# Alandroid/img-compression-mps

Measured on AMD Instinct MI355X. Metric: Mvoxels/s compress+reconstruct, 256^3 fp32, bond chi=64; SSIM vs ref, higher is better.
Workload: dtype f32

## Files before the change

img-compression-mps_amd/_lib.py:

```python
import ctypes as C
import os

_HERE = os.path.dirname(os.path.abspath(__file__))
LIB_PATH = os.path.join(_HERE, "libndmps_hip.so")

OK, EINVAL, EHIP, ENOCONV, EWORKSPACE, ETEAM = 0, -1, -2, -3, -4, -5

i64 = C.c_int64
p_i64 = C.POINTER(C.c_int64)
p_f64 = C.POINTER(C.c_double)
p_f32 = C.POINTER(C.c_float)
p_int = C.POINTER(C.c_int)
vp = C.c_void_p

SIGNATURES = {
    "ndmps_version": (C.c_int, []),
    "ndmps_last_error": (C.c_char_p, []),
    "ndmps_device_count": (C.c_int, []),
    "ndmps_streams_create": (C.c_int, [C.c_int, C.POINTER(vp), C.POINTER(C.c_int)]),
    "ndmps_streams_destroy": (C.c_int, [C.c_int, C.POINTER(vp)]),
    "ndmps_profile_enable": (C.c_int, [C.c_int]),
    "ndmps_profile_collect": (C.c_int, [C.c_int, p_f64, p_i64, p_i64]),
    "ndmps_plan_create": (C.c_int, [C.POINTER(vp), C.c_int, p_i64, C.c_int, p_i64]),
    "ndmps_plan_create_reversed": (C.c_int, [C.POINTER(vp), C.c_int, p_i64, C.c_int, p_i64]),
# ... 92 lines not shown
    "ndmps_potrf_scratch_elems": (i64, [i64]),
    "ndmps_potrf_lower_f64": (C.c_int, [vp, i64, vp, C.POINTER(C.c_int), vp]),
    "ndmps_syevd_topk_workspace_bytes": (i64, [i64, C.c_int, i64]),
    "ndmps_syevd_topk_stamps_offset": (i64, [i64, C.c_int, i64]),
    "ndmps_syevd_topk_values_f64": (C.c_int, [C.c_int, vp, i64, p_i64, vp, i64, vp, i64, i64, vp, i64, vp]),
    "ndmps_syevd_topk_vectors_f64": (C.c_int, [C.c_int, p_i64, p_i64, i64, vp, i64, p_int, vp]),
    "ndmps_syevd_topk_vectors_auto_f64": (C.c_int, [C.c_int, p_i64, i64, C.c_double, vp, vp, i64, vp, vp, i64, vp]),
    "ndmps_syevd_topk_recover_f64": (C.c_int, [C.c_int, p_i64, i64, vp, i64, p_int, vp]),
    "ndmps_syevd_topk_set_team": (C.c_int, [C.c_int]),
    "ndmps_syevd_topk_set_streamed": (C.c_int, [C.c_int]),
    "ndmps_syevd_topk_team_fallbacks": (i64, []),
    "ndmps_syevd_topk_team_slots": (C.c_int, [i64]),
    "ndmps_syevd_topk_note_team_fallback": (C.c_int, []),
    "ndmps_debug_inject_team_abort": (C.c_int, [C.c_int]),
    "ndmps_debug_lane_sums_f64": (C.c_int, [vp, vp, vp]),
    "ndmps_tt_sweep_pads_cores": (C.c_int, [C.c_int, p_i64, i64]),
    "ndmps_tt_sweep_async_ints": (i64, [C.c_int, C.c_int]),
    "ndmps_tt_sweep_async_doubles": (i64, [C.c_int, C.c_int, p_i64, i64]),
    "ndmps_tt_sweep_batched_fused_begin_f32": (C.c_int, [C.c_int, C.POINTER(vp), C.c_int, p_i64, C.c_double, i64,
                                                         C.POINTER(vp), p_i64, p_i64, vp, vp, vp, vp, vp, i64,
                                                         vp, i64, vp, vp, vp]),
    "ndmps_tt_sweep_finish": (C.c_int, [C.c_int, C.c_int, p_i64, i64, vp, vp, p_i64, p_f64, p_i64]),
    "ndmps_tt_sweep_batched_workspace_bytes": (i64, [C.c_int, C.c_int, p_i64, i64]),
    "ndmps_tt_sweep_batched_f32": (C.c_int, [C.c_int, C.POINTER(vp), C.c_int, p_i64, C.c_double, i64,
                                             C.POINTER(vp), p_i64, p_i64, p_f64, p_i64, vp, i64, vp]),
    "ndmps_tt_layout": (C.c_int, [C.c_int, p_i64, i64, p_i64, p_i64, p_i64, p_i64]),
    "ndmps_tt_sweep_f32": (C.c_int, [vp, C.c_int, p_i64, C.c_double, i64, vp, p_i64, p_i64, p_f64,
                                     p_i64, vp, i64, vp]),
    "ndmps_compress_bond_workspace_bytes": (i64, [i64, i64, i64, i64, i64]),
    "ndmps_compress_bond_f32": (C.c_int, [vp, vp, i64, i64, i64, i64, i64, C.c_double, i64, vp, vp,
# ... 102 lines not shown
```

img-compression-mps_amd/csrc/gemm.hip:

```cpp
#include <stdlib.h>

#include <algorithm>

#include <mutex>
#include <type_traits>

#include "common.h"

namespace {

typedef float f32x16 __attribute__((ext_vector_type(16)));
typedef double f64x4 __attribute__((ext_vector_type(4)));

template <typename T>
struct Mfma;

template <>
struct Mfma<float> {
  static constexpr int MT = 32;
  static constexpr int KS = 2;
  static constexpr int NACC = 16;
  typedef f32x16 acc_t;
  static __device__ __forceinline__ acc_t mma(float a, float b, acc_t c) {
    return __builtin_amdgcn_mfma_f32_32x32x2f32(a, b, c, 0, 0, 0);
// ... 829 lines not shown
    Gb[pr * n + pc] = s;
    Gb[pc * n + pr] = s;
  }
}

constexpr int G128_LD = 128 + 16;
constexpr int G128_PANEL = GW_KB * G128_LD;
constexpr size_t kGram128Lds = (size_t)4 * G128_PANEL * sizeof(float);
constexpr int kGram128MaxBatch = 48;

struct Gram128Geom {
  int tiles_1d, n_off, n_diag;
  int slabs_off, slabs_diag;
  int64_t rows_off, rows_diag;
  int slots;
  int xcd, members, groups_per_matrix, groups_total;
};
struct Gram128Ptrs {
  const void* a[kGram128MaxBatch];
};

template <int ROLE>
__device__ __forceinline__ void gram128_load(const float* pa, const float* pb, int s, double (&av)[4], double (&bv)[4]) {
  const int off = 4 * s * G128_LD;
  if (ROLE == 1) {
#pragma unroll
    for (int a = 0; a < 4; ++a) av[a] = bv[a] = (double)pa[off + 16 * a];
  } else {
#pragma unroll
    for (int a = 0; a < (ROLE == 2 ? 2 : 4); ++a) av[a] = (double)pa[off + 16 * a];
#pragma unroll
    for (int b = 0; b < 4; ++b) bv[b] = (double)pb[off + 16 * b];
  }
}
template <int ROLE>
// ... 3 lines not shown
#pragma unroll
    for (int b = 0; b < 4; ++b)
      if (ROLE != 1 || a <= b) acc[4 * a + b] = __builtin_amdgcn_mfma_f64_16x16x4f64(av[a], bv[b], acc[4 * a + b], 0, 0, 0);
}
template <int ROLE>
__device__ __forceinline__ void gram128_chunk(const float* pa, const float* pb, f64x4 (&acc)[16]) {
  double av[2][4], bv[2][4];
  gram128_load<ROLE>(pa, pb, 0, av[0], bv[0]);
#pragma unroll
  for (int s = 0; s < GW_KB / 4; ++s) {
    if (s + 1 < GW_KB / 4) gram128_load<ROLE>(pa, pb, s + 1, av[(s + 1) & 1], bv[(s + 1) & 1]);
    gram128_mfma<ROLE>(av[s & 1], bv[s & 1], acc);
  }
}

template <typename TIN, int MODE>
__global__ void __launch_bounds__(256, 2)
gram128_kernel(Gram128Ptrs ptrs, int64_t m, int64_t n, int64_t lda, double* __restrict__ partial, Gram128Geom g,
               int vec_ok, const int64_t* __restrict__ row_off, const int64_t* __restrict__ col_off) {
  extern __shared__ __attribute__((aligned(16))) float g128_lds[];
  int id = blockIdx.x, vol = blockIdx.y;
  if (g.xcd) {
    const int x = blockIdx.x & 7, q = blockIdx.x >> 3;
    const int group = (q / g.members) * 8 + x, mem = q % g.members;
    if (group >= g.groups_total) return;
    vol = group / g.groups_per_matrix;
    const int sp = group % g.groups_per_matrix;
    if (g.xcd == 2) {
      id = mem < g.n_off ? mem * g.slabs_off + sp : g.n_off * g.slabs_off + (mem - g.n_off) * g.slabs_diag + sp;
    } else if (mem < 2 * g.n_off) {
      const int sl = 2 * sp + mem / g.n_off;
      if (sl >= g.slabs_off) return;
      id = (mem % g.n_off) * g.slabs_off + sl;
    } else {
      id = g.n_off * g.slabs_off + (mem - 2 * g.n_off) * g.slabs_diag + sp;
    }
  }
  const TIN* __restrict__ A = static_cast<const TIN*>(ptrs.a[vol]);
  int ti, tj, slab;
  int64_t rows;
  if (id < g.n_off * g.slabs_off) {
    int t = id / g.slabs_off;
    slab = id % g.slabs_off;
    rows = g.rows_off;
    ti = 0;
    while (t >= g.tiles_1d - 1 - ti) {
      t -= g.tiles_1d - 1 - ti;
      ++ti;
    }
    tj = ti + 1 + t;
  } else {
    const int t = (id - g.n_off * g.slabs_off) / g.slabs_diag;
    slab = (id - g.n_off * g.slabs_off) % g.slabs_diag;
    rows = g.rows_diag;
    ti = tj = t;
  }
  const bool diag = ti == tj;
  const int64_t i0 = (int64_t)ti * 128, j0 = (int64_t)tj * 128;
  const int64_t r_begin = (int64_t)slab * rows;
  const int64_t r_end = min(m, r_begin + rows);

  const int tid = threadIdx.x, lane = tid & 63, wave = tid >> 6;
  const int lr = lane >> 4, lc = lane & 15;

  float4 pi[4], pj[4];
  int64_t coli = 0, colj = 0, ro[4] = {0, 0, 0, 0};
  auto row_offsets = [&](int64_t r0) {
    if (MODE == 2 || (MODE == 0 && row_off)) {
#pragma unroll
      for (int v = 0; v < 4; ++v) {
        const int64_t row = r0 + (tid + 256 * v) / 32;
        ro[v] = row < r_end ? row_off[row] : 0;
      }
    }
  };
  if (MODE == 2 || (MODE == 0 && row_off)) {
    const int c4 = (tid % 32) * 4;
    if (i0 + c4 + 3 < n) coli = col_off[i0 + c4];
    if (j0 + c4 + 3 < n) colj = col_off[j0 + c4];
  }
  auto fetch = [&](int64_t r0) {
    if constexpr (MODE != 0) {
      const int c4 = (tid % 32) * 4;
#pragma unroll
      for (int v = 0; v < 4; ++v) {
        const TIN* src = MODE == 2 ? A + ro[v] + coli : A + (r0 + (tid + 256 * v) / 32) * lda + i0 + c4;
        pi[v] = load4_as_f32(src);
      }
      if (!diag) {
#pragma unroll
        for (int v = 0; v < 4; ++v) {
          const TIN* src = MODE == 2 ? A + ro[v] + colj : A + (r0 + (tid + 256 * v) / 32) * lda + j0 + c4;
          pj[v] = load4_as_f32(src);
        }
      }
      return;
    }
#pragma unroll
    for (int v = 0; v < 4; ++v) {
      const int e = tid + 256 * v;
      const int rr = e / 32, c4 = (e % 32) * 4;
      const int64_t row = r0 + rr;
      float4 x = make_float4(0.f, 0.f, 0.f, 0.f), y = x;
      if (row < r_end && row_off) {
        const TIN* base = A + ro[v];
        if (i0 + c4 + 3 < n) x = load4_as_f32(base + coli);
        if (!diag && j0 + c4 + 3 < n) y = load4_as_f32(base + colj);
      } else if (row < r_end) {
        const TIN* base = A + row * lda;
        if (vec_ok && i0 + c4 + 3 < n) x = load4_as_f32(base + i0 + c4);
        else {
          if (i0 + c4 + 0 < n) x.x = (float)base[i0 + c4 + 0];
// ... 102 lines not shown
    base = g.n_off * g.slabs_off + (t - g.n_off) * g.slabs_diag;
    count = g.slabs_diag;
  }
  const int64_t r = (int64_t)ti * 128 + e / 128, c = (int64_t)tj * 128 + e % 128;
  if (r >= n || c >= n || (ti == tj && c < r)) return;
  const double* src = partial + ((int64_t)blockIdx.z * g.slots + base) * (128 * 128) + e;
  double s = 0.0;
  int sl = 0;
  for (; sl + 4 <= count; sl += 4) {
    const double v0 = src[(int64_t)(sl + 0) * 16384], v1 = src[(int64_t)(sl + 1) * 16384];
    const double v2 = src[(int64_t)(sl + 2) * 16384], v3 = src[(int64_t)(sl + 3) * 16384];
    s = (((s + v0) + v1) + v2) + v3;
  }
  for (; sl < count; ++sl) s += src[(int64_t)sl * 16384];
  double* Gb = G + (int64_t)blockIdx.z * stride_G;
  const int64_t pr = perm ? perm[r] : r, pc = perm ? perm[c] : c;
  Gb[pr * n + pc] = s;
  Gb[pc * n + pr] = s;
}

template <typename TIN>
__global__ void __launch_bounds__(256)
gram_small_kernel(const TIN* __restrict__ A, int64_t m, int n, int64_t lda, double* __restrict__ partial,
                  int vec_ok) {
  __shared__ double red[4][36];
  double acc[36];
#pragma unroll
  for (int i = 0; i < 36; ++i) acc[i] = 0.0;
  const int64_t stride = (int64_t)gridDim.x * 256;
  for (int64_t r = (int64_t)blockIdx.x * 256 + threadIdx.x; r < m; r += stride) {
// ... 338 lines not shown
inline bool gram_use_128(int64_t m, int64_t n) { return n >= 128 && m >= 256; }

Gram128Geom gram128_geometry(int64_t m, int64_t n, int batch) {
  Gram128Geom g;
  g.tiles_1d = (int)ndmps::ceil_div(n, 128);
  g.n_off = g.tiles_1d * (g.tiles_1d - 1) / 2;
  g.n_diag = g.tiles_1d;
  const double weight = g.n_off + 0.625 * g.n_diag;
  const double want = 2.0 * ndmps::kNumCU * (batch > 1 ? 12.0 : 1.0) / std::max(batch, 1) / weight;
  const int64_t floor_rows = batch > 1 ? 512 : 128;
  int64_t s_off = std::max<int64_t>(1, std::min<int64_t>((int64_t)(want + 0.5), std::max<int64_t>(m / floor_rows, 1)));
  g.rows_off = ndmps::round_up(ndmps::ceil_div(m, s_off), GW_KB);
  g.rows_diag = ndmps::round_up((g.rows_off * 8 + 4) / 5, GW_KB);
  g.slabs_off = (int)ndmps::ceil_div(m, g.rows_off);
  g.slabs_diag = (int)ndmps::ceil_div(m, g.rows_diag);
  g.xcd = 0;
  g.members = g.groups_per_matrix = g.groups_total = 0;
  const char* xe = getenv("NDMPS_GRAM_XCD");
  const int xmode = xe ? atoi(xe) : 0;
  if (batch > 1 && g.tiles_1d >= 2 && g.slabs_off >= 4 && xmode == 1) {
    g.rows_diag = 2 * g.rows_off;
    g.slabs_diag = (int)ndmps::ceil_div(m, g.rows_diag);
    g.xcd = 1;
    g.members = 2 * g.n_off + g.n_diag;
    g.groups_per_matrix = g.slabs_diag;
    g.groups_total = batch * g.groups_per_matrix;
  } else if (batch > 1 && g.tiles_1d >= 2 && g.slabs_off >= 4 && xmode == 2) {
    const int64_t s2 = std::max<int64_t>(1, (int64_t)(g.slabs_off * weight / (g.n_off + g.n_diag) + 0.5));
    g.rows_off = g.rows_diag = ndmps::round_up(ndmps::ceil_div(m, s2), GW_KB);
    g.slabs_off = g.slabs_diag = (int)ndmps::ceil_div(m, g.rows_off);
    g.xcd = 2;
    g.members = g.n_off + g.n_diag;
    g.groups_per_matrix = g.slabs_off;
    g.groups_total = batch * g.groups_per_matrix;
  }
  g.slots = g.n_off * g.slabs_off + g.n_diag * g.slabs_diag;
  return g;
}

inline int64_t gram128_workspace(int64_t m, int64_t n, int batch) {
  return (int64_t)batch * gram128_geometry(m, n, batch).slots * 128 * 128 * (int64_t)sizeof(double) + 256;
}

int gram128_opt_in() {
  static std::mutex mu;
  static bool done[64] = {};
  int dev = 0;
  NDMPS_CHECK_HIP(hipGetDevice(&dev));
  std::lock_guard<std::mutex> lock(mu);
  if (dev < 0 || dev >= 64 || done[dev]) return NDMPS_OK;
#define NDMPS_GRAM128_OPT_IN(T, MODE)                                                                          \
  NDMPS_CHECK_HIP(hipFuncSetAttribute(reinterpret_cast<const void*>(&gram128_kernel<T, MODE>),                 \
                                      hipFuncAttributeMaxDynamicSharedMemorySize, (int)kGram128Lds))
  NDMPS_GRAM128_OPT_IN(float, 0);
  NDMPS_GRAM128_OPT_IN(float, 1);
  NDMPS_GRAM128_OPT_IN(float, 2);
  NDMPS_GRAM128_OPT_IN(__bf16, 0);
  NDMPS_GRAM128_OPT_IN(__bf16, 1);
  NDMPS_GRAM128_OPT_IN(__bf16, 2);
#undef NDMPS_GRAM128_OPT_IN
  done[dev] = true;
  return NDMPS_OK;
}

template <typename TIN>
int gram128_batched(int batch, const TIN* const* h_A, int64_t m, int64_t n, int64_t lda, double* d_G, int64_t stride_G,
                    void* d_ws, int64_t ws_bytes, hipStream_t s, const int64_t* d_row_off, const int64_t* d_col_off,
                    const int32_t* d_perm = nullptr) {
  NDMPS_REQUIRE(batch >= 1 && h_A && d_G && gram_use_128(m, n) && lda >= n && stride_G >= n * n,
                "bad batched Gram argument (batch=%d m=%lld n=%lld)", batch, (long long)m, (long long)n);
  const int64_t need = gram128_workspace(m, n, batch);
  if (!d_ws || ws_bytes < need) {
    ndmps::set_error("Gram workspace too small: %lld < %lld", (long long)ws_bytes, (long long)need);
    return NDMPS_EWORKSPACE;
  }
  NDMPS_TRY(gram128_opt_in());
  const Gram128Geom g = gram128_geometry(m, n, batch);
  int vec_ok = (lda % 4 == 0 && n % 4 == 0) ? 1 : 0;
  for (int b = 0; b < batch; ++b) {
    NDMPS_REQUIRE(h_A[b], "NULL Gram operand %d", b);
    if ((uintptr_t)h_A[b] % (4 * sizeof(TIN)) != 0) vec_ok = 0;
  }
  if (d_row_off)
    NDMPS_REQUIRE(d_col_off && vec_ok, "gathered Gram needs n %% 4 == 0 and aligned bases");
  double* partial = (double*)d_ws;
  const bool turn = (int64_t)batch * g.slots >= 4096 && !getenv("NDMPS_GRAM_NO_TURN");
  static const bool one_turn = getenv("NDMPS_ONE_TURN") != nullptr;
  ndmps::Turn gram_turn(s, one_turn ? ndmps::kTurnTeam : ndmps::kTurnGram, one_turn ? 2u : 1u, one_turn ? 2u : 1u);
  if (turn) NDMPS_TRY(gram_turn.begin());
  void* span = ndmps::span_begin(s);
  for (int base = 0; base < batch; base += kGram128MaxBatch) {
    const int count = std::min(kGram128MaxBatch, batch - base);
    Gram128Ptrs ptrs;
    for (int t = 0; t < count; ++t) ptrs.a[t] = h_A[base + t];
    const bool interior = vec_ok && n % 128 == 0 && m % GW_KB == 0 && g.rows_off % GW_KB == 0 && g.rows_diag % GW_KB == 0 &&
                          !getenv("NDMPS_GRAM_GENERAL");
    auto kernel = !interior ? gram128_kernel<TIN, 0> : (d_row_off ? gram128_kernel<TIN, 2> : gram128_kernel<TIN, 1>);
    if (g.xcd) {
      Gram128Geom gc = g;
      gc.groups_total = count * g.groups_per_matrix;
      const unsigned wgs = (unsigned)(ndmps::ceil_div(gc.groups_total, 8) * g.members * 8);
      hipLaunchKernelGGL(kernel, dim3(wgs), dim3(256), kGram128Lds, s, ptrs, m, n, lda,
                         partial + (int64_t)base * g.slots * 16384, gc, vec_ok, d_row_off, d_col_off);
    } else {
      hipLaunchKernelGGL(kernel, dim3(g.slots, count), dim3(256), kGram128Lds, s, ptrs, m, n, lda,
                         partial + (int64_t)base * g.slots * 16384, g, vec_ok, d_row_off, d_col_off);
    }
  }
  ndmps::span_end(span, s, turn ? ndmps::kSpanGram : ndmps::kSpanGramSmall, (batch + kGram128MaxBatch - 1) / kGram128MaxBatch,
                  (int64_t)batch * m * n * (n + 1));
  NDMPS_TRY(gram_turn.end());
  hipLaunchKernelGGL(gram128_reduce_kernel, dim3(g.n_off + g.n_diag, 64, batch), dim3(256), 0, s, partial, g, d_G, stride_G, n,
                     d_perm);
  NDMPS_LAUNCH_CHECK();
  return NDMPS_OK;
}

extern "C" int64_t ndmps_gram_workspace_bytes(int64_t m, int64_t n) {
  if (m <= 0 || n <= 0) return 0;
  if (gram_use_small(n)) return (int64_t)kGramSmallBlocks * 36 * 8 + 256;
  if (gram_use_128(m, n)) return gram128_workspace(m, n, 1);
  if (gram_use_wide(m, n)) {
    GramGeom g = gram_wide_geometry(m, n);
    const int64_t ts = gram_wide_tile(n);
    return (int64_t)(g.n_slabs + g.n_slabs / kReduceGroup + 2) * g.n_tiles * ts * ts * (int64_t)sizeof(double) + 256;
  }
  GramGeom g = gram_geometry(m, n);
  const int ts = 16 * g.T;
// ... 127 lines not shown
  ndmps::span_end(span, s, ndmps::kSpanGramSmall, (batch + 63) / 64, (int64_t)batch * m * n * (n + 1));
  NDMPS_LAUNCH_CHECK();
  return NDMPS_OK;
}
}

extern "C" int64_t ndmps_gram_batched_workspace_bytes(int batch, int64_t m, int64_t n) {
  if (batch <= 0) return 0;
  if (gram_use_128(m, n)) return gram128_workspace(m, n, batch);
  if (gram_use_wide_batched(batch, m, n)) {
    const GramWideBatchGeom g = gram_wide_batched_geometry(batch, m, n);
    return (int64_t)batch * g.n_slabs * g.n_tiles * 4096 * 8 + 256;
  }
  return 0;
}
extern "C" int ndmps_gram_batched_f32(int batch, const float* const* h_A, int64_t m, int64_t n, int64_t lda,
                                      double* d_G, int64_t stride_G, void* d_ws, int64_t ws_bytes,
                                      ndmps_stream_t stream) {
  if (!gram_use_128(m, n) && gram_use_wide_batched(batch, m, n))
    return gram_wide_batched<float>(batch, h_A, m, n, lda, d_G, stride_G, d_ws, ws_bytes, (hipStream_t)stream, nullptr, nullptr,
                                    nullptr);
  return gram128_batched<float>(batch, h_A, m, n, lda, d_G, stride_G, d_ws, ws_bytes, (hipStream_t)stream, nullptr, nullptr);
}
extern "C" int ndmps_gram_batched_bf16(int batch, const void* const* h_A, int64_t m, int64_t n, int64_t lda,
                                       double* d_G, int64_t stride_G, void* d_ws, int64_t ws_bytes,
                                       ndmps_stream_t stream) {
  if (!gram_use_128(m, n) && gram_use_wide_batched(batch, m, n))
    return gram_wide_batched<__bf16>(batch, (const __bf16* const*)h_A, m, n, lda, d_G, stride_G, d_ws, ws_bytes,
                                     (hipStream_t)stream, nullptr, nullptr, nullptr);
  return gram128_batched<__bf16>(batch, (const __bf16* const*)h_A, m, n, lda, d_G, stride_G, d_ws, ws_bytes,
// ... 54 lines not shown
```

img-compression-mps_amd/csrc/tt.hip:

```cpp
#include <math.h>
#include <stdlib.h>

#include <algorithm>
#include <vector>

#include "common.h"
#include "trunc.h"

namespace {

constexpr double kCutoffFloor = 1e-6;
constexpr double kCutoffFloorF64 = 1e-8;
template <typename T>
constexpr double cutoff_floor() { return sizeof(T) == 8 ? kCutoffFloorF64 : kCutoffFloor; }
constexpr double kSweepEigTol = 1e-13;

inline double sweep_eig_tol(bool f64_storage = false) {
  const char* e = getenv("NDMPS_SWEEP_EIG_TOL");
  if (e) {
    const double v = atof(e);
    if (v >= 1e-16 && v <= 1e-6) return v;
  }
  return f64_storage ? 1e-15 : kSweepEigTol;
}
// ... 100 lines not shown
__global__ void __launch_bounds__(256) f32_to_f64_batched_kernel(BatchOps ops, int64_t n, double* __restrict__ y, int64_t y_stride) {
  const T* x = static_cast<const T*>(ops.in[blockIdx.y]);
  double* yb = y + (int64_t)blockIdx.y * y_stride;
  for (int64_t i = (int64_t)blockIdx.x * 256 + threadIdx.x; i < n; i += (int64_t)gridDim.x * 256) yb[i] = ndmps::to_f64(x[i]);
}
template <typename T>
__global__ void __launch_bounds__(256)
core_from_vectors_batched_kernel(const double* __restrict__ V, int64_t v_stride, int64_t n, int64_t k, BatchOps ops) {
  const double* Vb = V + (int64_t)blockIdx.y * v_stride;
  T* core = static_cast<T*>(ops.out[blockIdx.y]);
  const int64_t total = k * n;
  for (int64_t e = (int64_t)blockIdx.x * 256 + threadIdx.x; e < total; e += (int64_t)gridDim.x * 256) {
    const int64_t i = e / n, c = e % n;
    core[e] = ndmps::from_f64<T>(Vb[c * n + i]);
  }
}
__global__ void __launch_bounds__(256)
sqrt_clamp_batched_kernel(const double* __restrict__ w, int64_t stride, int64_t n, double* __restrict__ sg) {
  const double* wb = w + (int64_t)blockIdx.y * stride;
  double* sb = sg + (int64_t)blockIdx.y * stride;
  for (int64_t i = (int64_t)blockIdx.x * 256 + threadIdx.x; i < n; i += (int64_t)gridDim.x * 256) sb[i] = sqrt(fmax(wb[i], 0.0));
}
template <typename T>
__global__ void __launch_bounds__(256)
scale_cols_to_f32_batched_kernel(const double* __restrict__ M, int64_t m_stride, int64_t rows, int64_t ldm, int64_t k,
                                 const double* __restrict__ sigma, int64_t s_stride, double power, BatchOps ops) {
  const double* Mb = M + (int64_t)blockIdx.y * m_stride;
  const double* sb = sigma + (int64_t)blockIdx.y * s_stride;
  T* out = static_cast<T*>(ops.out[blockIdx.y]);
  const int64_t total = rows * k;
// ... 919 lines not shown
        hipLaunchKernelGGL(sqrt_clamp_kernel, dim3(grid1d(small)), dim3(256), 0, s, wb, small, sigb);
        hipLaunchKernelGGL(scale_cols_to_f32_kernel<T>, dim3(grid1d(m * k)), dim3(256), 0, s, Vb, m, m, k, sigb, 1.0,
                           nxt[b]);
        NDMPS_LAUNCH_CHECK();
        NDMPS_TRY(ndmps_dgemm(1, 0, k, n, m, Vb, m, Ab, n, UtA, n, s));
        hipLaunchKernelGGL(scale_rows_to_f32_kernel<T>, dim3(grid1d(k * n)), dim3(256), 0, s, UtA, k, n, sigb, -1.0,
                           core);
        NDMPS_LAUNCH_CHECK();
      }
      std::swap(cur[b], nxt[b]);
      cur_elems[b] = m * k;
      chi_r[b] = k;
      h_bonds_out[(int64_t)b * (L + 1) + i] = k;
    }
  }
  for (int b = 0; b < batch; ++b)
    NDMPS_CHECK_HIP(hipMemcpyAsync(h_cores[b] + h_core_offsets[0], cur[b], cur_elems[b] * sizeof(T),
                                   hipMemcpyDeviceToDevice, s));
  if (dev_rank && L > 1) {
    const size_t n_i = (size_t)2 * L * batch, n_s = (size_t)L * batch * lay.spec_stride;
    if (async) {
      NDMPS_REQUIRE(async->h_ranks && (async->h_spec || n_s == 0), "asynchronous sweep without its host buffers");
      NDMPS_CHECK_HIP(hipMemcpyAsync(async->h_ranks, d_ranks, n_i * sizeof(int), hipMemcpyDeviceToHost, s));
      if (n_s) NDMPS_CHECK_HIP(hipMemcpyAsync(async->h_spec, d_spec, n_s * sizeof(double), hipMemcpyDeviceToHost, s));
      return NDMPS_OK;
    }
    std::vector<int> host_i(n_i);
    std::vector<double> host_s(n_s);
    NDMPS_CHECK_HIP(hipMemcpyAsync(host_i.data(), d_ranks, n_i * sizeof(int), hipMemcpyDeviceToHost, s));
    if (n_s) NDMPS_CHECK_HIP(hipMemcpyAsync(host_s.data(), d_spec, n_s * sizeof(double), hipMemcpyDeviceToHost, s));
    NDMPS_CHECK_HIP(hipStreamSynchronize(s));
    return sweep_collect(batch, L, lay.spec_stride, host_i.data(), n_s ? host_s.data() : nullptr, h_bonds_out, h_spectra,
                         h_spec_offsets);
// ... 756 lines not shown
```

include/ndmps_hip.h:

```cpp
#ifndef NDMPS_HIP_H
#define NDMPS_HIP_H

#include <stdint.h>

#ifdef __cplusplus
extern "C" {
#endif

#define NDMPS_OK 0
#define NDMPS_EINVAL (-1)
#define NDMPS_EHIP (-2)
#define NDMPS_ENOCONV (-3)
#define NDMPS_EWORKSPACE (-4)
#define NDMPS_ETEAM (-5)

typedef void* ndmps_stream_t;
typedef struct ndmps_plan ndmps_plan_t;

int ndmps_version(void);
const char* ndmps_last_error(void);
int ndmps_device_count(void);

int ndmps_streams_create(int n, void** h_streams, int* n_independent);
int ndmps_streams_destroy(int n, void* const* h_streams);
// ... 121 lines not shown
int ndmps_potrf_lower_f64(double* d_S, int64_t n, double* d_scratch, int* h_status, ndmps_stream_t stream);
int ndmps_syevd_topk_values_f64(int batch, const double* d_G, int64_t stride_G, const int64_t* h_n,
                                double* d_V, int64_t stride_V, double* d_w, int64_t stride_w,
                                int64_t k_max, void* d_ws, int64_t ws_bytes, ndmps_stream_t stream);
int ndmps_syevd_topk_vectors_f64(int batch, const int64_t* h_n, const int64_t* h_k, int64_t k_max,
                                 void* d_ws, int64_t ws_bytes, int* h_status, ndmps_stream_t stream);
int ndmps_syevd_topk_recover_f64(int batch, const int64_t* h_n, int64_t k_max, void* d_ws, int64_t ws_bytes,
                                 int* h_recovered, ndmps_stream_t stream);
int ndmps_syevd_topk_set_team(int enabled);
int ndmps_syevd_topk_set_streamed(int streamed);
int64_t ndmps_syevd_topk_team_fallbacks(void);
int ndmps_syevd_topk_team_slots(int64_t order);
int ndmps_syevd_topk_note_team_fallback(void);
int ndmps_debug_inject_team_abort(int launches);
int ndmps_debug_lane_sums_f64(const double* d_in, double* d_out, ndmps_stream_t stream);
int ndmps_syevd_topk_vectors_auto_f64(int batch, const int64_t* h_n, int64_t k_cap, double cutoff,
                                      int* d_ranks, double* d_spectra, int64_t spectra_stride,
                                      int* d_status, void* d_ws, int64_t ws_bytes, ndmps_stream_t stream);

int ndmps_tt_layout(int L, const int64_t* h_dims, int64_t max_bond, int64_t* h_max_bonds,
                    int64_t* h_core_offsets, int64_t* h_spec_offsets,
                    int64_t* h_workspace_bytes);
int ndmps_tt_sweep_f32(float* d_dense, int L, const int64_t* h_dims, double cutoff,
                       int64_t max_bond, float* d_cores, const int64_t* h_core_offsets,
                       int64_t* h_bonds_out, double* h_spectra, const int64_t* h_spec_offsets,
                       void* d_ws, int64_t ws_bytes, ndmps_stream_t stream);

int ndmps_tt_sweep_pads_cores(int L, const int64_t* h_dims, int64_t max_bond);
int64_t ndmps_tt_sweep_async_ints(int batch, int L);
int64_t ndmps_tt_sweep_async_doubles(int batch, int L, const int64_t* h_dims, int64_t max_bond);
// ... 171 lines not shown
```

Measured before the change: 42450.

## Replace Gram128 slab grid with persistent stream-K walk and balanced schedule

After: 40160. 5.4% lower.

```diff
diff --git a/img-compression-mps_amd/_lib.py b/img-compression-mps_amd/_lib.py
--- a/img-compression-mps_amd/_lib.py
+++ b/img-compression-mps_amd/_lib.py
@@ -130,6 +130,7 @@
     "ndmps_syevd_topk_note_team_fallback": (C.c_int, []),
     "ndmps_debug_inject_team_abort": (C.c_int, [C.c_int]),
     "ndmps_debug_lane_sums_f64": (C.c_int, [vp, vp, vp]),
+    "ndmps_debug_gram128_schedule": (C.c_int, [i64, i64, C.c_int, C.c_int, C.c_int, p_i64, p_i64, C.c_int, p_i64]),
     "ndmps_tt_sweep_pads_cores": (C.c_int, [C.c_int, p_i64, i64]),
     "ndmps_tt_sweep_async_ints": (i64, [C.c_int, C.c_int]),
     "ndmps_tt_sweep_async_doubles": (i64, [C.c_int, C.c_int, p_i64, i64]),
diff --git a/img-compression-mps_amd/csrc/gemm.hip b/img-compression-mps_amd/csrc/gemm.hip
--- a/img-compression-mps_amd/csrc/gemm.hip
+++ b/img-compression-mps_amd/csrc/gemm.hip
@@ -1,6 +1,10 @@
 #include <stdlib.h>
 
 #include <algorithm>
+#include <cstring>
+#include <map>
+#include <tuple>
+#include <vector>
 
 #include <mutex>
 #include <type_traits>
@@ -867,11 +871,97 @@
   int slabs_off, slabs_diag;
   int64_t rows_off, rows_diag;
   int slots;
-  int xcd, members, groups_per_matrix, groups_total;
 };
 struct Gram128Ptrs {
   const void* a[kGram128MaxBatch];
 };
+constexpr int kGram128MaxGrid = 1024;
+struct Gram128Sched {
+  int tiles_1d, n_off, n_tiles;
+  int chunks;
+  int count, grid;
+  int slot_by_wg;
+  int64_t w_off, w_matrix, w_total;
+  unsigned char adj[kGram128MaxGrid / 2];
+};
+constexpr int kGram128WOff = 16, kGram128WDiag = 10;
+__host__ __device__ inline int64_t gram128_sched_base(const Gram128Sched& sc, int w) {
+  const int64_t per_matrix = (int64_t)sc.n_tiles * sc.chunks;
+  if (w >= sc.grid) return sc.count * per_matrix;
+  const int64_t t = (int64_t)w * sc.w_total / sc.grid;
+  const int64_t b = t / sc.w_matrix, rho = t % sc.w_matrix;
+  const int64_t r = rho < sc.w_off ? (rho + kGram128WOff / 2) / kGram128WOff
+                                   : (int64_t)sc.n_off * sc.chunks + (rho - sc.w_off + kGram128WDiag / 2) / kGram128WDiag;
+  return b * per_matrix + r;
+}
+__host__ __device__ inline int64_t gram128_sched_begin(const Gram128Sched& sc, int w) {
+  if (w >= sc.grid) return (int64_t)sc.count * sc.n_tiles * sc.chunks;
+  return gram128_sched_base(sc, w) + (int)((sc.adj[w >> 1] >> (4 * (w & 1))) & 15) - 8;
+}
+__host__ __device__ inline int64_t gram128_sched_slot(const Gram128Sched& sc, int w, int64_t tg) {
+  if (!sc.slot_by_wg) return w + tg;
+  return 2 * (int64_t)w + (tg * sc.chunks > gram128_sched_begin(sc, w) ? 1 : 0);
+}
+inline int64_t gram128_sched_slots(const Gram128Sched& sc) {
+  return sc.grid < 2 ? 0 : (sc.slot_by_wg ? 2 * (int64_t)sc.grid : (int64_t)sc.grid + (int64_t)sc.count * sc.n_tiles - 1);
+}
+inline int64_t gram128_sched_weight(const Gram128Sched& sc, int64_t u) {
+  const int64_t per_matrix = (int64_t)sc.n_tiles * sc.chunks, off_units = (int64_t)sc.n_off * sc.chunks;
+  const int64_t b = u / per_matrix, r = u % per_matrix;
+  return b * sc.w_matrix + (r <= off_units ? r * kGram128WOff : sc.w_off + (r - off_units) * kGram128WDiag);
+}
+inline bool gram128_balance(Gram128Sched& sc) {
+  memset(sc.adj, 0x88, sizeof(sc.adj));
+  const int g = sc.grid;
+  if (g < 2) return true;
+  constexpr int D = 7, ND = 2 * D + 1;
+  const int64_t units = (int64_t)sc.count * sc.n_tiles * sc.chunks;
+  std::vector<int64_t> wt((size_t)(g + 1) * ND, -1);
+  for (int w = 0; w <= g; ++w)
+    for (int d = 0; d < ND; ++d) {
+      if ((w == 0 || w == g) && d != D) continue;
+      const int64_t u = gram128_sched_base(sc, w) + d - D;
+      if (u >= 0 && u <= units) wt[(size_t)w * ND + d] = gram128_sched_weight(sc, u);
+    }
+  const int64_t share = sc.w_total / g;
+  std::vector<signed char> from((size_t)(g + 1) * ND);
+  for (int64_t lo = share; lo >= std::max<int64_t>(1, share - kGram128WOff); --lo) {
+    std::fill(from.begin(), from.end(), (signed char)-1);
+    from[D] = D;
+    for (int w = 1; w <= g; ++w)
+      for (int d = 0; d < ND; ++d) {
+        const int64_t here = wt[(size_t)w * ND + d];
+        if (here < 0) continue;
+        for (int e = 0; e < ND; ++e) {
+          if (from[(size_t)(w - 1) * ND + e] < 0) continue;
+          const int64_t x = here - wt[(size_t)(w - 1) * ND + e];
+          if (x >= lo && x <= lo + kGram128WOff) {
+            from[(size_t)w * ND + d] = (signed char)e;
+            break;
+          }
+        }
+      }
+    if (from[(size_t)g * ND + D] < 0) continue;
+    for (int w = g, d = D; w >= 1; --w) {
+      if (w < g) sc.adj[w >> 1] = (unsigned char)((sc.adj[w >> 1] & ~(15 << (4 * (w & 1)))) | ((d - D + 8) << (4 * (w & 1))));
+      d = from[(size_t)w * ND + d];
+    }
+    return true;
+  }
+  return false;
+}
+__host__ __device__ inline void gram128_tile(int tiles_1d, int n_off, int t, int& ti, int& tj) {
+  if (t >= n_off) {
+    ti = tj = t - n_off;
+    return;
+  }
+  ti = 0;
+  while (t >= tiles_1d - 1 - ti) {
+    t -= tiles_1d - 1 - ti;
+    ++ti;
+  }
+  tj = ti + 1 + t;
+}
 
 template <int ROLE>
 __device__ __forceinline__ void gram128_load(const float* pa, const float* pb, int s, double (&av)[4], double (&bv)[4]) {
@@ -905,28 +995,12 @@
   }
 }
 
-template <typename TIN, int MODE>
+template <typename TIN>
 __global__ void __launch_bounds__(256, 2)
-gram128_kernel(Gram128Ptrs ptrs, int64_t m, int64_t n, int64_t lda, double* __restrict__ partial, Gram128Geom g,
-               int vec_ok, const int64_t* __restrict__ row_off, const int64_t* __restrict__ col_off) {
+gram128_general_kernel(Gram128Ptrs ptrs, int64_t m, int64_t n, int64_t lda, double* __restrict__ partial, Gram128Geom g,
+                       int vec_ok, const int64_t* __restrict__ row_off, const int64_t* __restrict__ col_off) {
   extern __shared__ __attribute__((aligned(16))) float g128_lds[];
-  int id = blockIdx.x, vol = blockIdx.y;
-  if (g.xcd) {
-    const int x = blockIdx.x & 7, q = blockIdx.x >> 3;
-    const int group = (q / g.members) * 8 + x, mem = q % g.members;
-    if (group >= g.groups_total) return;
-    vol = group / g.groups_per_matrix;
-    const int sp = group % g.groups_per_matrix;
-    if (g.xcd == 2) {
-      id = mem < g.n_off ? mem * g.slabs_off + sp : g.n_off * g.slabs_off + (mem - g.n_off) * g.slabs_diag + sp;
-    } else if (mem < 2 * g.n_off) {
-      const int sl = 2 * sp + mem / g.n_off;
-      if (sl >= g.slabs_off) return;
-      id = (mem % g.n_off) * g.slabs_off + sl;
-    } else {
-      id = g.n_off * g.slabs_off + (mem - 2 * g.n_off) * g.slabs_diag + sp;
-    }
-  }
+  const int id = blockIdx.x, vol = blockIdx.y;
   const TIN* __restrict__ A = static_cast<const TIN*>(ptrs.a[vol]);
   int ti, tj, slab;
   int64_t rows;
@@ -957,7 +1031,7 @@
   float4 pi[4], pj[4];
   int64_t coli = 0, colj = 0, ro[4] = {0, 0, 0, 0};
   auto row_offsets = [&](int64_t r0) {
-    if (MODE == 2 || (MODE == 0 && row_off)) {
+    if (row_off) {
 #pragma unroll
       for (int v = 0; v < 4; ++v) {
         const int64_t row = r0 + (tid + 256 * v) / 32;
@@ -965,28 +1039,12 @@
       }
     }
   };
-  if (MODE == 2 || (MODE == 0 && row_off)) {
+  if (row_off) {
     const int c4 = (tid % 32) * 4;
     if (i0 + c4 + 3 < n) coli = col_off[i0 + c4];
     if (j0 + c4 + 3 < n) colj = col_off[j0 + c4];
   }
   auto fetch = [&](int64_t r0) {
-    if constexpr (MODE != 0) {
-      const int c4 = (tid % 32) * 4;
-#pragma unroll
-      for (int v = 0; v < 4; ++v) {
-        const TIN* src = MODE == 2 ? A + ro[v] + coli : A + (r0 + (tid + 256 * v) / 32) * lda + i0 + c4;
-        pi[v] = load4_as_f32(src);
-      }
-      if (!diag) {
-#pragma unroll
-        for (int v = 0; v < 4; ++v) {
-          const TIN* src = MODE == 2 ? A + ro[v] + colj : A + (r0 + (tid + 256 * v) / 32) * lda + j0 + c4;
-          pj[v] = load4_as_f32(src);
-        }
-      }
-      return;
-    }
 #pragma unroll
     for (int v = 0; v < 4; ++v) {
       const int e = tid + 256 * v;
@@ -1119,6 +1177,176 @@
   }
   for (; sl < count; ++sl) s += src[(int64_t)sl * 16384];
   double* Gb = G + (int64_t)blockIdx.z * stride_G;
+  const int64_t pr = perm ? perm[r] : r, pc = perm ? perm[c] : c;
+  Gb[pr * n + pc] = s;
+  Gb[pc * n + pr] = s;
+}
+
+template <typename TIN, int MODE>
+__global__ void __launch_bounds__(256, 2)
+gram128_kernel(Gram128Ptrs ptrs, int64_t n, int64_t lda, Gram128Sched sc, double* __restrict__ partial,
+               double* __restrict__ G, int64_t stride_G, const int64_t* __restrict__ row_off,
+               const int64_t* __restrict__ col_off, const int32_t* __restrict__ perm) {
+  static_assert(MODE == 1 || MODE == 2, "the persistent walk serves interior shapes only");
+  extern __shared__ __attribute__((aligned(16))) float g128_lds[];
+  const int tid = threadIdx.x, lane = tid & 63, wave = tid >> 6;
+  const int lr = lane >> 4, lc = lane & 15;
+  const int c4 = (tid % 32) * 4;
+  const int64_t u_end = gram128_sched_begin(sc, blockIdx.x + 1);
+  for (int64_t u = gram128_sched_begin(sc, blockIdx.x); u < u_end;) {
+    const int64_t tg = u / sc.chunks;
+    const int c_begin = (int)(u % sc.chunks);
+    const int c_end = (int)min((int64_t)sc.chunks, c_begin + (u_end - u));
+    u += c_end - c_begin;
+    const int vol = (int)(tg / sc.n_tiles);
+    int ti, tj;
+    gram128_tile(sc.tiles_1d, sc.n_off, (int)(tg % sc.n_tiles), ti, tj);
+    const bool diag = ti == tj;
+    const bool whole = c_begin == 0 && c_end == sc.chunks;
+    const TIN* __restrict__ A = static_cast<const TIN*>(ptrs.a[vol]);
+    const int64_t i0 = (int64_t)ti * 128, j0 = (int64_t)tj * 128;
+    const int64_t r_begin = (int64_t)c_begin * GW_KB, r_end = (int64_t)c_end * GW_KB;
+
+    float4 pi[4], pj[4];
+    int64_t coli = 0, colj = 0, ro[4] = {0, 0, 0, 0};
+    auto row_offsets = [&](int64_t r0) {
+      if (MODE == 2 && r0 < r_end) {
+#pragma unroll
+        for (int v = 0; v < 4; ++v) ro[v] = (row_off + r0 + 8 * v)[tid / 32];
+      }
+    };
+    if (MODE == 2) {
+      coli = col_off[i0 + c4];
+      colj = col_off[j0 + c4];
+    }
+    const uint32_t lane_off = (uint32_t)(tid / 32) * (uint32_t)lda + c4;
+    auto fetch = [&](int64_t r0) {
+#pragma unroll
+      for (int v = 0; v < 4; ++v) {
+        const TIN* src = MODE == 2 ? A + ro[v] + coli : A + (r0 + 8 * v) * lda + i0 + lane_off;
+        pi[v] = load4_as_f32(src);
+      }
+      if (!diag) {
+#pragma unroll
+        for (int v = 0; v < 4; ++v) {
+          const TIN* src = MODE == 2 ? A + ro[v] + colj : A + (r0 + 8 * v) * lda + j0 + lane_off;
+          pj[v] = load4_as_f32(src);
+        }
+      }
+    };
+    auto stash = [&](int buf) {
+      float* Pi = g128_lds + (2 * buf) * G128_PANEL;
+      float* Pj = Pi + G128_PANEL;
+#pragma unroll
+      for (int v = 0; v < 4; ++v) {
+        const int rr = (tid + 256 * v) / 32;
+        *reinterpret_cast<float4*>(Pi + rr * G128_LD + c4) = pi[v];
+        if (!diag) *reinterpret_cast<float4*>(Pj + rr * G128_LD + c4) = pj[v];
+      }
+    };
+
+    int a_col, b_col;
+    if (!diag) {
+      a_col = (wave >> 1) * 64;
+      b_col = (wave & 1) * 64;
+    } else if (wave == 0 || wave == 3) {
+      a_col = b_col = wave == 0 ? 0 : 64;
+    } else {
+      a_col = wave == 1 ? 0 : 32;
+      b_col = 64;
+    }
+    double* out = partial + gram128_sched_slot(sc, blockIdx.x, tg) * (128 * 128);
+    double* Gb = G + (int64_t)vol * stride_G;
+    auto run = [&](auto role_tag) {
+      constexpr int ROLE = decltype(role_tag)::value;
+      f64x4 acc[16];
+#pragma unroll
+      for (int a = 0; a < 16; ++a) acc[a] = (f64x4){0.0, 0.0, 0.0, 0.0};
+      row_offsets(r_begin);
+      fetch(r_begin);
+      stash(0);
+      row_offsets(r_begin + GW_KB);
+      __syncthreads();
+      int buf = 0;
+      for (int64_t r0 = r_begin; r0 < r_end; r0 += GW_KB, buf ^= 1) {
+        const bool more = r0 + GW_KB < r_end;
+        if (more) {
+          fetch(r0 + GW_KB);
+          row_offsets(r0 + 2 * GW_KB);
+        }
+        const float* Pi = g128_lds + (2 * buf) * G128_PANEL + lr * G128_LD + lc;
+        const float* Pj = ROLE == 0 ? Pi + G128_PANEL : Pi;
+        gram128_chunk<ROLE>(Pi + a_col, Pj + b_col, acc);
+        if (more) stash(buf ^ 1);
+        __syncthreads();
+      }
+      int t2 = tid;
+      asm volatile("" : "+v"(t2));
+      const int lr = (t2 & 63) >> 4, lc = t2 & 15, w2 = t2 >> 6;
+      const int a_col = !diag ? (w2 >> 1) * 64 : (w2 == 0 ? 0 : w2 == 3 ? 64 : w2 == 1 ? 0 : 32);
+      const int b_col = !diag ? (w2 & 1) * 64 : (w2 == 0 ? 0 : 64);
+      if (!whole) {
+#pragma unroll
+        for (int a = 0; a < (ROLE == 2 ? 2 : 4); ++a)
+#pragma unroll
+          for (int b = 0; b < 4; ++b) {
+            if (ROLE == 1 && a > b) continue;
+#pragma unroll
+            for (int reg = 0; reg < 4; ++reg)
+              out[(a_col + 16 * a + lr + 4 * reg) * 128 + b_col + 16 * b + lc] = acc[4 * a + b][reg];
+          }
+        return;
+      }
+      int pc[4];
+#pragma unroll
+      for (int b = 0; b < 4; ++b) {
+        const int c = (int)j0 + b_col + 16 * b + lc;
+        pc[b] = perm ? perm[c] : c;
+      }
+#pragma unroll
+      for (int a = 0; a < (ROLE == 2 ? 2 : 4); ++a)
+#pragma unroll
+        for (int reg = 0; reg < 4; ++reg) {
+          const int r = (int)i0 + a_col + 16 * a + lr + 4 * reg;
+          const int pr = perm ? perm[r] : r;
+#pragma unroll
+          for (int b = 0; b < 4; ++b) {
+            if (ROLE == 1 && a > b) continue;
+            if (ROLE == 1 && a == b && lc < lr + 4 * reg) continue;
+            Gb[(int64_t)pr * n + pc[b]] = acc[4 * a + b][reg];
+            Gb[(int64_t)pc[b] * n + pr] = acc[4 * a + b][reg];
+          }
+        }
+    };
+    if (!diag) run(std::integral_constant<int, 0>{});
+    else if (wave == 0 || wave == 3) run(std::integral_constant<int, 1>{});
+    else run(std::integral_constant<int, 2>{});
+  }
+}
+
+__global__ void __launch_bounds__(256)
+gram128_fixup_kernel(const double* __restrict__ partial, Gram128Sched sc, double* __restrict__ G, int64_t stride_G, int64_t n,
+                     const int32_t* __restrict__ perm) {
+  const int tg = blockIdx.x;
+  auto owner = [&](int64_t u) {
+    int lo = 0, hi = sc.grid - 1;
+    while (lo < hi) {
+      const int mid = (lo + hi + 1) / 2;
+      if (gram128_sched_begin(sc, mid) <= u) lo = mid;
+      else hi = mid - 1;
+    }
+    return lo;
+  };
+  const int w_first = owner((int64_t)tg * sc.chunks), w_last = owner((int64_t)(tg + 1) * sc.chunks - 1);
+  if (w_first == w_last) return;
+  const int e = blockIdx.y * 256 + threadIdx.x;
+  int ti, tj;
+  gram128_tile(sc.tiles_1d, sc.n_off, tg % sc.n_tiles, ti, tj);
+  const int64_t r = (int64_t)ti * 128 + e / 128, c = (int64_t)tj * 128 + e % 128;
+  if (ti == tj && c < r) return;
+  double s = 0.0;
+  for (int w = w_first; w <= w_last; ++w) s += partial[gram128_sched_slot(sc, w, tg) * (128 * 128) + e];
+  double* Gb = G + (int64_t)(tg / sc.n_tiles) * stride_G;
   const int64_t pr = perm ? perm[r] : r, pc = perm ? perm[c] : c;
   Gb[pr * n + pc] = s;
   Gb[pc * n + pr] = s;
@@ -1487,26 +1715,6 @@
   g.rows_diag = ndmps::round_up((g.rows_off * 8 + 4) / 5, GW_KB);
   g.slabs_off = (int)ndmps::ceil_div(m, g.rows_off);
   g.slabs_diag = (int)ndmps::ceil_div(m, g.rows_diag);
-  g.xcd = 0;
-  g.members = g.groups_per_matrix = g.groups_total = 0;
-  const char* xe = getenv("NDMPS_GRAM_XCD");
-  const int xmode = xe ? atoi(xe) : 0;
-  if (batch > 1 && g.tiles_1d >= 2 && g.slabs_off >= 4 && xmode == 1) {
-    g.rows_diag = 2 * g.rows_off;
-    g.slabs_diag = (int)ndmps::ceil_div(m, g.rows_diag);
-    g.xcd = 1;
-    g.members = 2 * g.n_off + g.n_diag;
-    g.groups_per_matrix = g.slabs_diag;
-    g.groups_total = batch * g.groups_per_matrix;
-  } else if (batch > 1 && g.tiles_1d >= 2 && g.slabs_off >= 4 && xmode == 2) {
-    const int64_t s2 = std::max<int64_t>(1, (int64_t)(g.slabs_off * weight / (g.n_off + g.n_diag) + 0.5));
-    g.rows_off = g.rows_diag = ndmps::round_up(ndmps::ceil_div(m, s2), GW_KB);
-    g.slabs_off = g.slabs_diag = (int)ndmps::ceil_div(m, g.rows_off);
-    g.xcd = 2;
-    g.members = g.n_off + g.n_diag;
-    g.groups_per_matrix = g.slabs_off;
-    g.groups_total = batch * g.groups_per_matrix;
-  }
   g.slots = g.n_off * g.slabs_off + g.n_diag * g.slabs_diag;
   return g;
 }
@@ -1515,24 +1723,73 @@
   return (int64_t)batch * gram128_geometry(m, n, batch).slots * 128 * 128 * (int64_t)sizeof(double) + 256;
 }
 
-int gram128_opt_in() {
+Gram128Sched gram128_schedule_uncached(int64_t m, int64_t n, int batch, int count, int resident) {
+  const Gram128Geom g = gram128_geometry(m, n, batch);
+  Gram128Sched sc;
+  sc.tiles_1d = g.tiles_1d;
+  sc.n_off = g.n_off;
+  sc.n_tiles = g.n_off + g.n_diag;
+  sc.chunks = (int)(m / GW_KB);
+  sc.count = count;
+  sc.w_off = (int64_t)sc.n_off * sc.chunks * kGram128WOff;
+  sc.w_matrix = sc.w_off + (int64_t)g.n_diag * sc.chunks * kGram128WDiag;
+  sc.w_total = sc.w_matrix * count;
+  const int64_t by_work = sc.w_total / ((batch > 1 ? 16 : 4) * kGram128WOff);
+  const int64_t by_tile = (int64_t)count * (g.slots - sc.n_tiles) + 1, by_wg = (int64_t)count * g.slots / 2;
+  sc.slot_by_wg = by_wg > by_tile ? 1 : 0;
+  const int64_t by_slots = std::max(by_tile, by_wg);
+  sc.grid = (int)std::max<int64_t>(1, std::min<int64_t>(std::min<int64_t>(std::min(resident, kGram128MaxGrid), by_work), by_slots));
+  const int widest = sc.grid;
+  bool ok = gram128_balance(sc);
+  while (!ok && sc.grid > 1 && sc.grid > widest - 32) {
+    --sc.grid;
+    ok = gram128_balance(sc);
+  }
+  if (!ok) {
+    sc.grid = widest;
+    gram128_balance(sc);
+  }
+  return sc;
+}
+Gram128Sched gram128_schedule_cached(int64_t m, int64_t n, int batch, int count, int resident) {
   static std::mutex mu;
-  static bool done[64] = {};
+  static std::map<std::tuple<int64_t, int64_t, int, int, int>, Gram128Sched> known;
+  std::lock_guard<std::mutex> lock(mu);
+  const auto key = std::make_tuple(m, n, batch, count, resident);
+  auto it = known.find(key);
+  if (it == known.end()) it = known.emplace(key, gram128_schedule_uncached(m, n, batch, count, resident)).first;
+  return it->second;
+}
+
+int gram128_opt_in(int* resident) {
+  static std::mutex mu;
+  static int done[64] = {};
   int dev = 0;
   NDMPS_CHECK_HIP(hipGetDevice(&dev));
+  NDMPS_REQUIRE(dev >= 0 && dev < 64, "device %d out of range", dev);
   std::lock_guard<std::mutex> lock(mu);
-  if (dev < 0 || dev >= 64 || done[dev]) return NDMPS_OK;
-#define NDMPS_GRAM128_OPT_IN(T, MODE)                                                                          \
-  NDMPS_CHECK_HIP(hipFuncSetAttribute(reinterpret_cast<const void*>(&gram128_kernel<T, MODE>),                 \
-                                      hipFuncAttributeMaxDynamicSharedMemorySize, (int)kGram128Lds))
-  NDMPS_GRAM128_OPT_IN(float, 0);
-  NDMPS_GRAM128_OPT_IN(float, 1);
-  NDMPS_GRAM128_OPT_IN(float, 2);
-  NDMPS_GRAM128_OPT_IN(__bf16, 0);
-  NDMPS_GRAM128_OPT_IN(__bf16, 1);
-  NDMPS_GRAM128_OPT_IN(__bf16, 2);
+  if (!done[dev]) {
+    int least = 1 << 30;
+#define NDMPS_GRAM128_OPT_IN(K)                                                                                  \
+  do {                                                                                                           \
+    int per_cu = 0;                                                                                              \
+    NDMPS_CHECK_HIP(hipFuncSetAttribute(reinterpret_cast<const void*>(&K), hipFuncAttributeMaxDynamicSharedMemorySize, \
+                                        (int)kGram128Lds));                                                      \
+    NDMPS_CHECK_HIP(hipOccupancyMaxActiveBlocksPerMultiprocessor(&per_cu, K, 256, kGram128Lds));                 \
+    least = std::min(least, per_cu);                                                                             \
+  } while (0)
+    NDMPS_GRAM128_OPT_IN(gram128_general_kernel<float>);
+    NDMPS_GRAM128_OPT_IN(gram128_general_kernel<__bf16>);
+    least = 1 << 30;
+    NDMPS_GRAM128_OPT_IN((gram128_kernel<float, 1>));
+    NDMPS_GRAM128_OPT_IN((gram128_kernel<float, 2>));
+    NDMPS_GRAM128_OPT_IN((gram128_kernel<__bf16, 1>));
+    NDMPS_GRAM128_OPT_IN((gram128_kernel<__bf16, 2>));
 #undef NDMPS_GRAM128_OPT_IN
-  done[dev] = true;
+    NDMPS_REQUIRE(least >= 1, "gram128_kernel does not fit a compute unit");
+    done[dev] = least * ndmps::kNumCU;
+  }
+  *resident = done[dev];
   return NDMPS_OK;
 }
 
@@ -1547,7 +1804,8 @@
     ndmps::set_error("Gram workspace too small: %lld < %lld", (long long)ws_bytes, (long long)need);
     return NDMPS_EWORKSPACE;
   }
-  NDMPS_TRY(gram128_opt_in());
+  int resident = 0;
+  NDMPS_TRY(gram128_opt_in(&resident));
   const Gram128Geom g = gram128_geometry(m, n, batch);
   int vec_ok = (lda % 4 == 0 && n % 4 == 0) ? 1 : 0;
   for (int b = 0; b < batch; ++b) {
@@ -1562,29 +1820,38 @@
   ndmps::Turn gram_turn(s, one_turn ? ndmps::kTurnTeam : ndmps::kTurnGram, one_turn ? 2u : 1u, one_turn ? 2u : 1u);
   if (turn) NDMPS_TRY(gram_turn.begin());
   void* span = ndmps::span_begin(s);
+  const bool interior = vec_ok && n % 128 == 0 && m % GW_KB == 0 && !getenv("NDMPS_GRAM_GENERAL");
   for (int base = 0; base < batch; base += kGram128MaxBatch) {
     const int count = std::min(kGram128MaxBatch, batch - base);
     Gram128Ptrs ptrs;
     for (int t = 0; t < count; ++t) ptrs.a[t] = h_A[base + t];
-    const bool interior = vec_ok && n % 128 == 0 && m % GW_KB == 0 && g.rows_off % GW_KB == 0 && g.rows_diag % GW_KB == 0 &&
-                          !getenv("NDMPS_GRAM_GENERAL");
-    auto kernel = !interior ? gram128_kernel<TIN, 0> : (d_row_off ? gram128_kernel<TIN, 2> : gram128_kernel<TIN, 1>);
-    if (g.xcd) {
-      Gram128Geom gc = g;
-      gc.groups_total = count * g.groups_per_matrix;
-      const unsigned wgs = (unsigned)(ndmps::ceil_div(gc.groups_total, 8) * g.members * 8);
-      hipLaunchKernelGGL(kernel, dim3(wgs), dim3(256), kGram128Lds, s, ptrs, m, n, lda,
-                         partial + (int64_t)base * g.slots * 16384, gc, vec_ok, d_row_off, d_col_off);
+    double* part = partial + (int64_t)base * g.slots * 16384;
+    if (interior) {
+      const Gram128Sched sc = gram128_schedule_cached(m, n, batch, count, resident);
+      NDMPS_REQUIRE(gram128_sched_slots(sc) <= (int64_t)count * g.slots, "internal: Gram partial slots outgrow the workspace");
+      auto kernel = d_row_off ? gram128_kernel<TIN, 2> : gram128_kernel<TIN, 1>;
+      hipLaunchKernelGGL(kernel, dim3(sc.grid), dim3(256), kGram128Lds, s, ptrs, n, lda, sc, part,
+                         d_G + (int64_t)base * stride_G, stride_G, d_row_off, d_col_off, d_perm);
     } else {
-      hipLaunchKernelGGL(kernel, dim3(g.slots, count), dim3(256), kGram128Lds, s, ptrs, m, n, lda,
-                         partial + (int64_t)base * g.slots * 16384, g, vec_ok, d_row_off, d_col_off);
+      hipLaunchKernelGGL(gram128_general_kernel<TIN>, dim3(g.slots, count), dim3(256), kGram128Lds, s, ptrs, m, n, lda, part, g,
+                         vec_ok, d_row_off, d_col_off);
     }
   }
   ndmps::span_end(span, s, turn ? ndmps::kSpanGram : ndmps::kSpanGramSmall, (batch + kGram128MaxBatch - 1) / kGram128MaxBatch,
                   (int64_t)batch * m * n * (n + 1));
   NDMPS_TRY(gram_turn.end());
-  hipLaunchKernelGGL(gram128_reduce_kernel, dim3(g.n_off + g.n_diag, 64, batch), dim3(256), 0, s, partial, g, d_G, stride_G, n,
-                     d_perm);
+  if (interior) {
+    for (int base = 0; base < batch; base += kGram128MaxBatch) {
+      const int count = std::min(kGram128MaxBatch, batch - base);
+      const Gram128Sched sc = gram128_schedule_cached(m, n, batch, count, resident);
+      if (sc.grid > 1)
+        hipLaunchKernelGGL(gram128_fixup_kernel, dim3(count * sc.n_tiles, 64), dim3(256), 0, s,
+                           partial + (int64_t)base * g.slots * 16384, sc, d_G + (int64_t)base * stride_G, stride_G, n, d_perm);
+    }
+  } else {
+    hipLaunchKernelGGL(gram128_reduce_kernel, dim3(g.n_off + g.n_diag, 64, batch), dim3(256), 0, s, partial, g, d_G, stride_G, n,
+                       d_perm);
+  }
   NDMPS_LAUNCH_CHECK();
   return NDMPS_OK;
 }
@@ -1742,6 +2009,29 @@
   }
   return 0;
 }
+extern "C" int ndmps_debug_gram128_schedule(int64_t m, int64_t n, int batch, int resident, int launch, int64_t* first,
+                                            int64_t* last, int cap, int64_t* info) {
+  NDMPS_REQUIRE(batch >= 1 && resident >= 1 && launch >= 0 && first && last && info, "bad schedule query");
+  NDMPS_REQUIRE(gram_use_128(m, n) && n % 128 == 0 && m % GW_KB == 0, "not an interior Gram shape (m=%lld n=%lld)", (long long)m,
+                (long long)n);
+  const int launches = (batch + kGram128MaxBatch - 1) / kGram128MaxBatch;
+  NDMPS_REQUIRE(launch < launches, "launch %d of %d", launch, launches);
+  const int count = std::min(kGram128MaxBatch, batch - launch * kGram128MaxBatch);
+  const Gram128Sched sc = gram128_schedule_cached(m, n, batch, count, resident);
+  NDMPS_REQUIRE(sc.grid <= cap, "schedule arrays too short: %d < %d", cap, sc.grid);
+  for (int w = 0; w < sc.grid; ++w) {
+    first[w] = gram128_sched_begin(sc, w);
+    last[w] = gram128_sched_begin(sc, w + 1) - 1;
+  }
+  info[0] = count;
+  info[1] = sc.n_tiles;
+  info[2] = sc.n_off;
+  info[3] = sc.chunks;
+  info[4] = launches;
+  info[5] = (int64_t)count * gram128_geometry(m, n, batch).slots;
+  info[6] = gram128_sched_slots(sc);
+  return sc.grid;
+}
 extern "C" int ndmps_gram_batched_f32(int batch, const float* const* h_A, int64_t m, int64_t n, int64_t lda,
                                       double* d_G, int64_t stride_G, void* d_ws, int64_t ws_bytes,
                                       ndmps_stream_t stream) {
diff --git a/img-compression-mps_amd/csrc/tt.hip b/img-compression-mps_amd/csrc/tt.hip
--- a/img-compression-mps_amd/csrc/tt.hip
+++ b/img-compression-mps_amd/csrc/tt.hip
@@ -138,6 +138,18 @@
     const int64_t i = e / n, c = e % n;
     core[e] = ndmps::from_f64<T>(Vb[c * n + i]);
   }
+}
+struct BatchCopy {
+  const void* in[kSmallBatch];
+  void* out[kSmallBatch];
+  int64_t n[kSmallBatch];
+};
+template <typename T>
+__global__ void __launch_bounds__(256) copy_batched_kernel(BatchCopy cp) {
+  const T* in = static_cast<const T*>(cp.in[blockIdx.y]);
+  T* out = static_cast<T*>(cp.out[blockIdx.y]);
+  const int64_t n = cp.n[blockIdx.y];
+  for (int64_t i = (int64_t)blockIdx.x * 256 + threadIdx.x; i < n; i += (int64_t)gridDim.x * 256) out[i] = in[i];
 }
 __global__ void __launch_bounds__(256)
 sqrt_clamp_batched_kernel(const double* __restrict__ w, int64_t stride, int64_t n, double* __restrict__ sg) {
@@ -1087,9 +1099,19 @@
       h_bonds_out[(int64_t)b * (L + 1) + i] = k;
     }
   }
-  for (int b = 0; b < batch; ++b)
-    NDMPS_CHECK_HIP(hipMemcpyAsync(h_cores[b] + h_core_offsets[0], cur[b], cur_elems[b] * sizeof(T),
-                                   hipMemcpyDeviceToDevice, s));
+  for (int base = 0; base < batch; base += kSmallBatch) {
+    const int count = std::min(kSmallBatch, batch - base);
+    BatchCopy cp;
+    int64_t longest = 0;
+    for (int b = 0; b < count; ++b) {
+      cp.in[b] = cur[base + b];
+      cp.out[b] = h_cores[base + b] + h_core_offsets[0];
+      cp.n[b] = cur_elems[base + b];
+      longest = std::max(longest, cp.n[b]);
+    }
+    hipLaunchKernelGGL(copy_batched_kernel<T>, dim3(grid1d(longest), count), dim3(256), 0, s, cp);
+    NDMPS_LAUNCH_CHECK();
+  }
   if (dev_rank && L > 1) {
     const size_t n_i = (size_t)2 * L * batch, n_s = (size_t)L * batch * lay.spec_stride;
     if (async) {
diff --git a/include/ndmps_hip.h b/include/ndmps_hip.h
--- a/include/ndmps_hip.h
+++ b/include/ndmps_hip.h
@@ -159,6 +159,8 @@
 int ndmps_syevd_topk_note_team_fallback(void);
 int ndmps_debug_inject_team_abort(int launches);
 int ndmps_debug_lane_sums_f64(const double* d_in, double* d_out, ndmps_stream_t stream);
+int ndmps_debug_gram128_schedule(int64_t m, int64_t n, int batch, int resident, int launch, int64_t* first, int64_t* last,
+                                 int cap, int64_t* info);
 int ndmps_syevd_topk_vectors_auto_f64(int batch, const int64_t* h_n, int64_t k_cap, double cutoff,
                                       int* d_ranks, double* d_spectra, int64_t spectra_stride,
                                       int* d_status, void* d_ws, int64_t ws_bytes, ndmps_stream_t stream);
```
